# areanddee/Sharding-the-Sphere-Fall-2025-JAX-DevLab-Examples

Measured on AMD Instinct MI355X. Metric: cell-updates/sec (whole node) at C96, higher is better.
Workload: dtype fp64; 1 GPU; global_batch=1, seq_len=55296, parallelism=spatial tiles: 24 tiles over 1 GPU(s), auto partition, N=96, tiles_per_edge=2, integrator=ssprk3, backend=hip, comm=none, steps_per_launch=6, fused_block=16, graph_replayed_steps=0, direct_launch_steps=1662, kernel_launches=277, eager_steps=0

## Files before the change

### sharding-the-sphere-fall-2025-jax-devlab-examples_amd/ops/csrc/fused_step.hip

```cpp
#include "stage_common.h"

#include <type_traits>


#ifndef STSP_FPROBE_ALLEDGE
#define STSP_FPROBE_ALLEDGE 0
#endif
#ifndef STSP_XG_FENCE
#define STSP_XG_FENCE 0
#endif
#ifndef STSP_FUSED_TAGH
#define STSP_FUSED_TAGH 1
#endif
#ifndef STSP_FUSED_TAIL_OWN
#define STSP_FUSED_TAIL_OWN 1
#endif
#ifndef STSP_FUSED_POLL2
#define STSP_FUSED_POLL2 1
#endif
#ifndef STSP_FUSED_RF_MINB
#define STSP_FUSED_RF_MINB 12
#endif

namespace {
// ... 10 lines not shown
  static constexpr int WW = GB + GMAX;
  static constexpr int L1 = R - 2 * (NS - 1);
  static constexpr int H1 = B + 4 * (NS - 1);
  static constexpr int NFX = H1 * (H1 + 1);
  static constexpr int NFL = 2 * NFX;
  static constexpr int NU = H1 * H1;
  static constexpr int NT = NU <= 768 ? 768 : 1024;
  static_assert(NU <= NT && W * W <= 2 * NT, "owner threads for every updated cell");
  static constexpr int NTAIL = W * W > NT ? W * W - NT : 0;
  static constexpr int NTO = STSP_FUSED_TAIL_OWN ? B * B : NT - NU;
  static constexpr int TPT = NTAIL ? (NTAIL + NTO - 1) / NTO : 1;
  static_assert(GMAX <= NT, "one fix-up thread per ghost entry");
  static_assert(2 * (B + 4 * (NS - 2)) * (B + 4 * (NS - 2) + 1) <= 32 * 64 && 2 * H1 * (H1 + 1) <= 32 * 64 + 64 * 64,
                "face passes per stage fit the 32-entry pass table");
  static constexpr int CMAX = 32;
};

__device__ __forceinline__ int fregion(int X, int Y, int N) {
  const bool inx = (unsigned)X < (unsigned)N, iny = (unsigned)Y < (unsigned)N;
  if (inx) return iny ? 0 : (Y < 0 ? 3 : 4);
  return iny ? (X < 0 ? 1 : 2) : -1;
}

__host__ __device__ __forceinline__ constexpr void annulus(int t, int lo, int L, int w, int& u, int& v) {
  if (t < w * L) {
    u = lo + t % L; v = lo + t / L;
    return;
  }
  t -= w * L;
  if (t < w * L) {
// ... 88 lines not shown
  unsigned mdiv_n;
  T a0[4], a1[4], a2[4];
  T dt, g, omega2;
  int ring, K;
  const unsigned long long* recv;
  T* const* peer_ring;
  const int* xpush;
  int* epoch;
  int* err;
  long long timeout_ticks;
  unsigned long long* stamps;
  int nsteps;
  const int* prod;
  int PM;
  const unsigned* sched;
  const T* nrmf;
  unsigned long long* hx;
  const signed char* pidx;
};

__device__ __forceinline__ void fused_fail(int* err, unsigned code, int bid, int xe, int what, int seen) {
  if (atomicCAS((unsigned*)err, 0u, code) == 0u) {
    __hip_atomic_store(err + 1, bid, __ATOMIC_RELAXED, __HIP_MEMORY_SCOPE_AGENT);
    __hip_atomic_store(err + 2, xe, __ATOMIC_RELAXED, __HIP_MEMORY_SCOPE_AGENT);
    __hip_atomic_store(err + 3, what, __ATOMIC_RELAXED, __HIP_MEMORY_SCOPE_AGENT);
    __hip_atomic_store(err + 4, seen, __ATOMIC_RELAXED, __HIP_MEMORY_SCOPE_AGENT);
  }
}

template <class C, int SCOPE, bool FENCE = false, class Fail>
// ... 82 lines not shown

template <typename T>
__device__ __forceinline__ T pair_swap(T v) {
  if constexpr (sizeof(T) == 8) {
    int2 p = __builtin_bit_cast(int2, v);
    p.x = __builtin_amdgcn_update_dpp(0, p.x, 0xB1, 0xF, 0xF, false);
    p.y = __builtin_amdgcn_update_dpp(0, p.y, 0xB1, 0xF, 0xF, false);
    return __builtin_bit_cast(T, p);
  } else {
    return __builtin_bit_cast(T, __builtin_amdgcn_update_dpp(0, __builtin_bit_cast(int, v), 0xB1, 0xF, 0xF, false));
  }
}

__device__ __forceinline__ int sel5(int r, int v0, int v1, int v2, int v3, int v4) {
  return r == 0 ? v0 : r == 1 ? v1 : r == 2 ? v2 : r == 3 ? v3 : v4;
}

__device__ __forceinline__ int ncode(unsigned long long c, int side) {
  return (int)(short)(unsigned short)(c >> (16 * side));
}

template <typename T, int LIM, int NS, int B, bool XG, bool MULTI>
__global__ __launch_bounds__((FD<NS, B>::NT)) void fused_step_kernel(FArgs<T> a) {
  using D = FD<NS, B>;
  constexpr int W = D::W, WS = D::WS, WW = D::WW, GB = D::GB, R = D::R, L1 = D::L1, H1 = D::H1;
  constexpr int NFX = D::NFX, NFL = D::NFL, NT = D::NT;
  static_assert(window_covered_once<NS, B>(), "owner and tail cells cover the window exactly once");
  constexpr bool RING_FIRST = B >= STSP_FUSED_RF_MINB;
  constexpr bool PFN = sizeof(T) == 4 || B <= 16;
  constexpr int NRG = PFN ? 1 : 5;
  constexpr int NN = 2 * NRG * 3 * (W + 1);
  __shared__ T s_w[5 * WW];
  __shared__ T s_fl[4][NFL];
  __shared__ T s_len[NFL];
  __shared__ T s_nrm[2][NRG][3][W + 1];
  __shared__ T s_nrmf[PFN ? 3 * NFL : 1];
  constexpr int CS = W + 1;
  __shared__ unsigned long long s_code[W * CS];
  __shared__ short s_gs[D::GMAX][2];
  __shared__ T s_gt[D::GMAX];
  __shared__ int s_ct[D::CMAX][CT_INTS];
  __shared__ T s_cg[D::CMAX][CG_VALS];
  constexpr int NX2 = NS > 1 ? (B + 4 * (NS - 2)) * (B + 4 * (NS - 2)) : 1;
  __shared__ T s_x[4][NX2];
  __shared__ int s_gdone;

  const int tid = threadIdx.x;
  const int bid = xcd_remap(blockIdx.x, a.nblocks);
  const int N = a.N;
  const int* og = a.org + bid * 4;
  const int X0 = og[0], Y0 = og[1], tile = og[2], ow = og[3];
  const int xo = ow & 0xFFF, yo = (ow >> 12) & 0xFFF, flags = (ow >> 24) & 0x1F;
  const bool edge = (flags & 0x1E) != 0;
  const int ngw = edge ? (a.G + 63) >> 6 : 0;
  int gbase = 0;
  int gtarget = 0;
  if (tid == 0) s_gdone = 0;
  const T* wf = &s_w[0];
  FSTAMP(0);
  FSTAMP_RT(14);
// ... 41 lines not shown
      gs1 = a.gtab[((long)bid * a.G + tid) * 2 + 1];
      gtv = a.gw[(long)bid * a.G + tid];
    }
    ncor = a.ccnt[bid];
    gbase = 64 * (ncor > 0 ? 1 : 0);
    if (tid < ncor) {
      const int* ct = a.ctab + ((long)bid * a.C + tid) * CT_INTS;
      const T* cg = a.cgf + ((long)bid * a.C + tid) * CG_VALS;
#pragma unroll
      for (int k = 0; k < CT_INTS; ++k) ctv[k] = ct[k];
#pragma unroll
      for (int k = 0; k < CG_VALS; ++k) cgv[k] = cg[k];
    }
  }
  const int wv = __builtin_amdgcn_readfirstlane(tid >> 6);
  unsigned pmask[3], nmask[3];
#pragma unroll
  for (int s = 0; s < 3; ++s) {
    pmask[s] = __builtin_amdgcn_readfirstlane(a.sched[((long)bid * 3 + s) * 17 + wv]);
    nmask[s] = __builtin_amdgcn_readfirstlane(a.sched[((long)bid * 3 + s) * 17 + 16]);
  }
  constexpr int LPT = (NFL + NT - 1) / NT;
  T lnv[LPT];
  if (flags == 1) {
#pragma unroll
    for (int k = 0; k < LPT; ++k) {
      const int j = tid + k * NT;
      const bool yf = j >= NFX;
      const int jj = yf ? j - NFX : j;
      const int r = yf ? jj / H1 : jj / (H1 + 1), c = yf ? jj - r * H1 : jj - r * (H1 + 1);
      const int li = yf ? (X0 + L1 + c) * (N + 1) + Y0 + L1 + r : (Y0 + L1 + r) * (N + 1) + X0 + L1 + c;
      lnv[k] = j < NFL ? a.lxt[li] : T(0);
    }
  } else {
#pragma unroll
// ... 138 lines not shown
      to_global((int)(a.frames >> (9 * ((unsigned)ow >> 29))) & 511, ax ? T(0) : rn, ax ? rn : T(0), -nrv * rn,
                m0, m1, m2);
      s_nrm[ax][0][0][k] = m0; s_nrm[ax][0][1][k] = m1; s_nrm[ax][0][2][k] = m2;
    } else {
      (&s_nrm[0][0][0][0])[tid] = nrv;
    }
  }
  if (!PFN && NN > NT && flags != 1 && tid + NT < NN) (&s_nrm[0][0][0][0])[tid + NT] = nrv2;
  if (PFN && flags != 1) {
#pragma unroll
    for (int k = 0; k < NPF; ++k) {
      const int j = tid + k * NT;
      if (j < 3 * NFL) s_nrmf[j] = nfv[k];
    }
  }
  if (edge) {
    if (owner) s_code[v * CS + u] = cdv;
    if (tid < a.G) { s_gs[tid][0] = (short)gs0; s_gs[tid][1] = (short)gs1; s_gt[tid] = gtv; }
    if (tid < ncor) {
#pragma unroll
      for (int k = 0; k < CT_INTS; ++k) s_ct[tid][k] = ctv[k];
#pragma unroll
      for (int k = 0; k < CG_VALS; ++k) s_cg[tid][k] = cgv[k];
    }
  }
  auto put_at = [&](int wi, const T (&q)[4]) {
    const T inv = q[0] != T(0) ? trcp(q[0]) : T(0);
    T* p = &s_w[0] + wi;
    p[0] = q[0];
    p[WW] = q[1] * inv;
// ... 72 lines not shown
      wl[f] = cl[f] + half_slope<LIM>(cl[f] - am, ap - cl[f]);
      wr[f] = cr[f] - half_slope<LIM>(cr[f] - bm, bp - cr[f]);
    }
    T m0, m1, m2;
    if constexpr (MODE != 0 && PFN) {
      m0 = s_nrmf[fslot]; m1 = s_nrmf[NFL + fslot]; m2 = s_nrmf[2 * NFL + fslot];
    } else {
      const T* m = &s_nrm[ax ? 1 : 0][ra][0][k];
      m0 = m[0]; m1 = m[W + 1]; m2 = m[2 * (W + 1)];
    }
    T fl[4];
    swe_flux<T>(wl, wr, cl, cr, m0, m1, m2, s_len[fslot], a.g, fl);
#pragma unroll
    for (int f = 0; f < 4; ++f) s_fl[f][fslot] = fl[f];
  };
  constexpr int NIL = B - 3, NI = 2 * NIL * B;
  constexpr int OL0 = R + 2 - L1, OL1 = (W - L1) - (R + B - 1) + 1;
  constexpr int NR1 = H1, NOR = H1 - B;
  constexpr int NOA = (OL0 + OL1) * NR1, NOX = NOA + NIL * NOR;
  static_assert(NOX + NIL * B == H1 * (H1 + 1), "inner + outer = the stage-1 face set");
  auto inner_face = [&](int t) {
    const bool ax = t >= NIL * B;
    const int t2 = ax ? t - NIL * B : t;
    const int k = R + 2 + t2 / B, p = R + t2 % B;
    if (PFN && edge) {
      if (ax) face(true, p, k, k, std::integral_constant<int, 1>{});
      else face(false, k, p, k, std::integral_constant<int, 1>{});
    } else {
      if (ax) face(true, p, k, k, std::integral_constant<int, 0>{});
      else face(false, k, p, k, std::integral_constant<int, 0>{});
// ... 16 lines not shown
      for (int f = 0; f < 4; ++f) s_x[f][tid] = Q[f];
    }
    if (owner) put(Q);
  };

  for (int it = 0; it < nsteps; ++it) {
  FSTAMP(13);
  const bool wait = MULTI && it > 0;
  if (wait) {
    if (tid < B * B) enter_cell();
  } else {
    enter_cell();
  }
  __syncthreads();
  if (wait && !tagh && !pcell && tid < 64) {
    const int p = tid < a.PM ? a.prod[(long)bid * a.PM + tid] : -1;
    const int pa = p >= 0 ? p : bid;
    bool ok = false;
    xg_spin(a.err, a.timeout_ticks, [&] {
      const int e = __hip_atomic_load(a.epoch + pa, __ATOMIC_RELAXED, __HIP_MEMORY_SCOPE_AGENT);
      ok = p < 0 || e >= xe;
      return __builtin_amdgcn_ballot_w64(!ok) == 0;
    }, [&] {
      if (!ok) fused_fail(a.err, 2u, bid, xe, p, __hip_atomic_load(a.epoch + p, __ATOMIC_RELAXED,
                                                                    __HIP_MEMORY_SCOPE_AGENT));
    });
  } else {
    const bool w0 = wait && !tagh && !pcell;
    const bool rf = RING_FIRST && wait && tagh;
    const int t0 = w0 ? tid - 64 : (rf ? (tid < B * B ? B * B - 1 - tid : NI) : tid);
    const int dt_ = w0 ? NT - 64 : (rf ? B * B : NT);
// ... 1 lines not shown
  }
  FSTAMP(1);
  if (!(wait && (tagh || pcell))) __syncthreads();
  if (wait) {
    T tq[TPT][4];
    if (tagh) {
      tail_load_tagged(xe, tq);
      if (tid >= B * B) {
        if (src >= 0) load_tagged(src, Q, xe);
        else load_state_of(src, Q, nullptr, xe);
        enter_cell();
      }
    } else {
      if (pcell) {
        auto poll_prod = [&](int cu, int cv) {
          const int k = a.pidx[(long)bid * W * W + cv * W + cu];
          if (k < 0) return;
          const int p = a.prod[(long)bid * a.PM + k];
          int e = 0;
          xg_spin(a.err, a.timeout_ticks, [&] {
            e = __hip_atomic_load(a.epoch + p, __ATOMIC_RELAXED, __HIP_MEMORY_SCOPE_AGENT);
            return e >= xe;
          }, [&] { fused_fail(a.err, 2u, bid, xe, p, e); });
        };
        if (tid >= B * B && owner) poll_prod(u, v);
#pragma unroll
        for (int k = 0; k < TPT; ++k)
          if (tl_wi[k] >= 0) poll_prod(tl_wi[k] % WS, tl_wi[k] / WS);
      }
      tail_load(buf[it & 1], xe, tq);
      if (tid >= B * B) {
// ... 21 lines not shown
          const T x0 = wf[f * WW + i0], x1 = wf[f * WW + i1];
          s_w[f * WW + GB + ge] = x0 + t * (x1 - x0);
        }
      }
      if (ge >= 0 && ge < ngw * 64 && (tid & 63) == 0) {
        asm volatile("s_waitcnt lgkmcnt(0)" ::: "memory");
        __hip_atomic_fetch_add(&s_gdone, 1, __ATOMIC_RELEASE, __HIP_MEMORY_SCOPE_WORKGROUP);
      }
      gtarget += ngw;
    }
    const int nax = s == 0 ? NOX : nx;
    const int ntask = 2 * nax;
    unsigned m = pmask[s];
    for (int first = (ncor && wv == 0) ? 1 : 0; first || m;) {
      int task;
      bool nearp = false;
      if (first) {
        task = (tid & 63) - 64;
        first = 0;
      } else {
        const int pp = __builtin_ctz(m);
        task = pp * 64 + (tid & 63);
        nearp = (nmask[s] >> pp) & 1u;
        m &= m - 1u;
      }
      if (task >= ntask) continue;
      if (task >= 0) {
        const int tf = task;
        const bool ax = tf >= nax;
        const int t2 = ax ? tf - nax : tf;
        int fu, fv, k, p;
        if (s == 0) {
          outer_face(t2, k, p);
        } else {
          const int c = t2 / nr, r = t2 - c * nr;
          k = lo + c; p = lo + r;
        }
        if (!ax) { fv = p; fu = k; }
        else { fu = p; fv = k; }
        if (edge || STSP_FPROBE_ALLEDGE) {
          if (PFN && !nearp) face(ax, fu, fv, k, std::integral_constant<int, 1>{});
          else face(ax, fu, fv, k, std::integral_constant<int, 2>{});
// ... 95 lines not shown
      for (int f = 0; f < 4; ++f) {
        T* p = o32(Out, so + f * S);
        if constexpr (sizeof(T) == 8)
          __hip_atomic_store((gu64*)p, __builtin_bit_cast(unsigned long long, Q[f]), __ATOMIC_RELAXED,
                             __HIP_MEMORY_SCOPE_AGENT);
        else
          __hip_atomic_store((gu32*)p, __builtin_bit_cast(unsigned, Q[f]), __ATOMIC_RELAXED,
                             __HIP_MEMORY_SCOPE_AGENT);
      }
    } else {
#pragma unroll
      for (int f = 0; f < 4; ++f) *o32(Out, so + f * S) = Q[f];
    }
    if (last) {
      const int n = a.n, mg = a.mg;
      const int x = xo + u - R, y = yo + v - R;
      const int* pm = a.push + (long)tile * 4 * mg * n;
      int pt[4] = {-1, -1, -1, -1};
      if (x < mg) pt[0] = pm[(0 * mg + x) * n + y];
      if (x >= n - mg) pt[1] = pm[(1 * mg + (n - 1 - x)) * n + y];
      if (y < mg) pt[2] = pm[(2 * mg + y) * n + x];
      if (y >= n - mg) pt[3] = pm[(3 * mg + (n - 1 - y)) * n + x];
      if (a.cpush && (x < mg || x >= n - mg) && (y < mg || y >= n - mg)) {
        const int qx = x < mg ? 0 : 1, qy = y < mg ? 0 : 1;
        const int c = a.cpush[((tile * 4 + (qx | (qy << 1))) * mg + (qy ? n - 1 - y : y)) * mg + (qx ? n - 1 - x : x)];
        if (c != -1) pt[qx ^ 1] = c;
      }
#pragma unroll
      for (int k = 0; k < 4; ++k) {
        if (pt[k] >= 0) {
#pragma unroll
// ... 53 lines not shown
    a.a0[k] = (T)d->a0[k]; a.a1[k] = (T)d->a1[k]; a.a2[k] = (T)d->a2[k];
  }
  a.dt = (T)d->dt; a.g = (T)d->g; a.omega2 = (T)d->omega2;
  a.ring = d->ring; a.K = d->K; a.recv = (const unsigned long long*)d->recv; a.peer_ring = (T* const*)d->peer_ring;
  a.xpush = d->xpush; a.epoch = d->epoch; a.err = d->err; a.timeout_ticks = d->timeout_ticks;
  a.stamps = d->stamps;
  for (int k = 0; k < 6; ++k) a.links[k] = d->links[k];
  a.local_src = d->local_src;
  a.nsteps = d->nsteps < 1 ? 1 : d->nsteps;
  a.prod = d->prod;
  a.PM = d->PM;
  a.sched = (const unsigned*)d->sched;
  a.nrmf = (const T*)d->nrmf;
  a.hx = (unsigned long long*)d->hx;
  a.pidx = d->pidx;
  if (!a.sched || !a.nrmf) return -4;
  if (a.nsteps > 1 && (!a.prod || a.PM <= 0 || a.PM > 64 || !d->epoch || !d->err)) return -7;
  a.mdiv_n = magic_div((unsigned)d->n, (unsigned long long)d->N + 1);
  if (d->xg && (!d->recv || !d->peer_ring || !d->xpush || !d->epoch || !d->err || d->ring <= 0 ||
                d->K <= 0))
    return -6;
  const dim3 grid(d->nblocks), block(D::NT);
  if (d->limiter < 0 || d->limiter > 3) return -4;
  if (a.nsteps > 1) {
    static int cdev[2][4] = {{-1, -1, -1, -1}, {-1, -1, -1, -1}}, ccap[2][4] = {};
    int dev = 0;
    if (hipGetDevice(&dev) != hipSuccess) return -8;
    const int xi = d->xg ? 1 : 0, li = d->limiter;
    if (cdev[xi][li] != dev) {
      int cus = 0, per = 0;
      if (hipDeviceGetAttribute(&cus, hipDeviceAttributeMultiprocessorCount, dev) != hipSuccess) return -8;
// ... 76 lines not shown
extern "C" int stsp_fused_prime_launch(int dtype, const void* q, int S, const int* src, const int* code, int nent,
                                       void* const* peer_ring, int ring, int epoch, hipStream_t stream) {
  if (nent <= 0) return 0;
  const dim3 grid((nent + 255) / 256), block(256);
  if (dtype == 1)
    hipLaunchKernelGGL(fused_prime_kernel<double>, grid, block, 0, stream, (const double*)q, S, src, code, nent,
                       (double* const*)peer_ring, ring, epoch);
  else if (dtype == 0)
    hipLaunchKernelGGL(fused_prime_kernel<float>, grid, block, 0, stream, (const float*)q, S, src, code, nent,
                       (float* const*)peer_ring, ring, epoch);
  else
    return -4;
  return (int)hipGetLastError();
}

extern "C" int stsp_fused_tagh(void) { return STSP_FUSED_TAGH; }

extern "C" int stsp_fused_limits(int* gmax, int* cmax) {
  *gmax = FD<3, 16>::GMAX;
  *cmax = FD<3, 16>::CMAX;
  return 0;
}
```

### sharding-the-sphere-fall-2025-jax-devlab-examples_amd/ops/csrc/stsp_kernels.h

```cpp
#pragma once
#include <hip/hip_runtime.h>
#include <stdint.h>

extern "C" {

typedef struct StageDesc {
  const void* X;
  const void* Q;
  const void* acc_in;
  void* out;
  void* acc_out;
  const void* recv;
  const int* gmap;
  const int* push;
  const int* blocks;
  const void* invA;
  const void* ex;
  const void* ey;
  const void* mx;
  const void* my;
  const void* cgeo;
  int ntile, n, S, mg, pw;
  int nblocks;
  int limiter;
// ... 73 lines not shown
  int K;
  int* epoch;
  int* err;
  long long timeout_ticks;
  unsigned long long* stamps;
  int local_src;
  int links[6];
  int nsteps;
  const int* prod;
  int PM;
  const int* cpush;
  const unsigned* sched;
  const void* nrmf;
  void* hx;
  const signed char* pidx;
} FusedDesc;
int stsp_fused_launch(int dtype, const FusedDesc* d, hipStream_t stream);
int stsp_fused_limits(int* gmax, int* cmax);
int stsp_fused_tagh(void);
int stsp_fused_record_words(int dtype);
int stsp_fused_prime_launch(int dtype, const void* q, int S, const int* src, const int* code, int nent,
                            void* const* peer_ring, int ring, int epoch, hipStream_t stream);
typedef struct DerivedDesc {
  const void* Q;
  const void* recv;
  const int* gmap;
  const int* cgmap;
  const int* pedge;
  const int* pe_base;
  const void* pe_t;
  const void* cdx;
  const void* cdy;
  const void* mx;
  const void* my;
// ... 180 lines not shown
```

### sharding-the-sphere-fall-2025-jax-devlab-examples_amd/ops/fused.py

```python
from __future__ import annotations

import hashlib
import os
from dataclasses import dataclass
from typing import Dict, List, Optional, Tuple

import numpy as np
import torch

from ..models.base import panel_edge_tables
from ..parallel.layout import TileLayout, ghost_xy
from ..parallel.topology import neighbor_cells


def native_stream(device) -> int:
    from .native import current_stream_handle
    return current_stream_handle(device)

REG_P, REG_W, REG_E, REG_S, REG_N = 0, 1, 2, 3, 4
NREG = 5
SIDE_VEC = ((-1, 0), (1, 0), (0, -1), (0, 1))
NG_PLR = 2


# ... 735 lines not shown


def stage_face_counts(B: int, ns: int = 3) -> List[int]:
    h1 = B + 4 * (ns - 1)
    nil = B - 3
    out = [2 * (h1 * (h1 + 1) - nil * B)]
    for s in range(1, ns):
        nr = B + 4 * (ns - 1 - s)
        out.append(2 * nr * (nr + 1))
    return out


PASS_SLOTS = 32


def pass_schedule(B: int, ncorner: np.ndarray, edge: np.ndarray, G: int, ns: int = 3,
                  weights: Optional[str] = None) -> np.ndarray:
    import os
    weights = weights or os.environ.get("STSP_FUSED_SCHED", "5:1")
    nt = fused_threads(B, ns)
    nw = nt // 64
    counts = stage_face_counts(B, ns)
    nb = len(ncorner)
    out = np.zeros((nb, ns, PASS_SLOTS), dtype=np.uint8)
    ngw = -(-G // 64) if G > 0 else 0
    cache = {}
    for b in range(nb):
        cw = 1 if ncorner[b] > 0 else 0
        gw = ngw if edge[b] else 0
        key = (cw, gw)
        if key not in cache:
            tab = np.zeros((ns, PASS_SLOTS), dtype=np.uint8)
            for s, nt_s in enumerate(counts):
                npass = -(-nt_s // 64)
                assert npass <= PASS_SLOTS
                if weights == "legacy":
                    first = nw - cw
                    for p in range(npass):
                        tab[s, p] = p + cw if p < first else cw + gw + (p - first) % (nw - cw - gw)
                    continue
                wc, wg = (int(x) for x in weights.split(":"))
                wl = [0] * nw
                if cw:
                    wl[0] += wc
                for w in range(cw, cw + gw):
                    wl[w] += wg
                for p in range(npass):
                    gl = [sum(wl[w] for w in range(g, nw, 4)) for g in range(4)]
                    g = min(range(4), key=lambda g_: (gl[g_], g_))
                    w = min(range(g, nw, 4), key=lambda w_: (wl[w_], w_))
                    tab[s, p] = w
                    wl[w] += 4
            cache[key] = tab
        out[b] = cache[key]
    return out


def pass_masks(B: int, sched: np.ndarray, ns: int = 3, near: Optional[np.ndarray] = None) -> np.ndarray:
    counts = stage_face_counts(B, ns)
    nb = sched.shape[0]
    m = np.zeros((nb, ns, 17), dtype=np.uint32)
    for s_, cnt in enumerate(counts):
        for p in range(-(-cnt // 64)):
            w = sched[:, s_, p].astype(np.int64)
            m[np.arange(nb), s_, w] |= np.uint32(1 << p)
    if near is not None:
        m[:, :, 16] = near
# ... 70 lines not shown
    fu = L1 + c
    fv = L1 + r
    k = np.where(yf, fv, fu)
    lu = fu - np.where(yf, 0, 1)
    lv = fv - np.where(yf, 1, 0)
    ax = yf.astype(np.int64)
    out = np.zeros((P.nb, 3, nfl))
    for b in range(P.nb):
        if flags[b] == 1:
            continue
        X0, Y0 = int(P.org[b, 0]), int(P.org[b, 1])
        ra = region(X0 + lu, Y0 + lv, P.N)
        ra = np.where(ra < 0, 0, ra)
        out[b] = P.nrm[b, ax, ra, k, :].T
    return out


def fused_supported(engine, B: Optional[int] = None) -> Optional[str]:
    e = engine
    return fused_supported_config(e.physics, e.integ.name, e.layout, B)


def fused_supported_config(physics, integrator: str, layout: TileLayout, B: Optional[int] = None) -> Optional[str]:
    from ..models.swe import ShallowWater
    if not isinstance(physics, ShallowWater):
        return "fused step: shallow water only"
    if getattr(physics, "kernel_id", None) == 4:
        return "fused step: no layers"
    if physics.F != 4:
        return "fused step: no tracers"
# ... 114 lines not shown
        if self.handoff == "tag" and not int(self.lib.stsp_fused_tagh()):
            if os.environ.get("STSP_FUSED_HANDOFF") == "tag":
                raise RuntimeError("STSP_FUSED_HANDOFF=tag needs a library built with STSP_FUSED_TAGH=1")
            self.handoff = "epoch"
        if self.handoff == "tag":
            words = 5 if e.dtype == torch.float64 else 4
            self.tens["hx"] = torch.zeros(2 * words * e.plan.S, dtype=torch.int64, device=dev)
        self.tens["err"] = torch.zeros(8, dtype=torch.int32, device=dev)
        prod = producer_table(P)
        self.tens["prod"] = torch.as_tensor(prod, dtype=torch.int32, device=dev).contiguous()
        self.poll = poll_mode() if (X is None and self.handoff == "epoch" and read_relation_symmetric(P)) \
            else "block"
        if self.poll == "cell":
            self.tens["pidx"] = torch.as_tensor(cell_producer_index(P, prod), device=dev).contiguous()
        edge_b = np.array([any(int(x) > 0 for x in np.unique(P.reg[b])) for b in range(nb)])
        sched = pass_schedule(B, np.asarray(P.ccnt), edge_b, G)
        assert int(sched.max()) < fused_threads(B) // 64
        flg = (org[:, 3].view(np.uint32) >> 24) & 0x1F
        near = near_pass_masks(B, P.org, flg.astype(np.int64), e.layout.N)
        self.tens["sched"] = torch.as_tensor(pass_masks(B, sched, near=near).view(np.int32), device=dev).contiguous()
        self.tens["nrmf"] = t(face_normals(P, flg.astype(np.int64)))
        self.timeout_ticks = int(timeout_s * 1e8)
        if X is not None:
            self._setup_exchange(X, timeout_s)
        self.descs = [self._desc(0, 1), self._desc(1, 0)]
        self._multi = {}
        self._multi_ptrs = {}
        if X is not None:
            self.prime()

    def _setup_exchange(self, X, timeout_s: float) -> None:
        from .xgmi import IpcRing, _declare, refuse_if_forced
        refuse_if_forced()
        e = self.e
        L = _declare(self.lib)
# ... 39 lines not shown
        d.dt = e.dt
        d.g = float(e.physics.g)
        d.omega2 = 2.0 * float(e.physics.omega)
        d.local_src = 1 if (self.world == 1 and not e.layout.loopback
                            and list(e.plan.tiles) == list(range(e.layout.num_tiles))) else 0
        for f in range(6):
            d.links[f] = face_links(f)
        d.epoch = p(tn["epoch"])
        d.err = p(tn["err"])
        d.timeout_ticks = self.timeout_ticks
        d.nsteps = nsteps
        d.prod = p(tn["prod"])
        d.PM = int(tn["prod"].shape[1])
        d.sched = p(tn["sched"])
        d.nrmf = p(tn["nrmf"])
        d.hx = p(tn["hx"]) if self.handoff == "tag" else 0
        d.pidx = p(tn["pidx"]) if self.poll == "cell" else 0
        if self.mem is not None:
            d.xg = 1
            d.ring = self.ring
            d.recv = self.mem.base
            d.peer_ring = p(tn["peer_ring"])
            d.xpush = p(tn["xpush"])
            d.K = self.K
        return d

    def multi_desc(self, nsteps: int):
        if nsteps < 2 or nsteps % 2:
            raise ValueError("a multi-step launch runs an even number of steps")
        d = self._multi.get(nsteps)
# ... 318 lines not shown
```

### sharding-the-sphere-fall-2025-jax-devlab-examples_amd/ops/native.py

```python
from __future__ import annotations

import ctypes
import os
import threading

import torch

from . import build as _build

_LIB = None
_LOCK = threading.Lock()


class StageDesc(ctypes.Structure):
    _fields_ = [
        ("X", ctypes.c_void_p), ("Q", ctypes.c_void_p), ("acc_in", ctypes.c_void_p),
        ("out", ctypes.c_void_p), ("acc_out", ctypes.c_void_p), ("recv", ctypes.c_void_p),
        ("gmap", ctypes.c_void_p), ("push", ctypes.c_void_p), ("blocks", ctypes.c_void_p),
        ("invA", ctypes.c_void_p), ("ex", ctypes.c_void_p), ("ey", ctypes.c_void_p),
        ("mx", ctypes.c_void_p), ("my", ctypes.c_void_p), ("cgeo", ctypes.c_void_p),
        ("ntile", ctypes.c_int), ("n", ctypes.c_int), ("S", ctypes.c_int), ("mg", ctypes.c_int), ("pw", ctypes.c_int),
        ("nblocks", ctypes.c_int), ("limiter", ctypes.c_int), ("remote", ctypes.c_int),
        ("a0", ctypes.c_double), ("a1", ctypes.c_double), ("a2", ctypes.c_double),
        ("c0", ctypes.c_double), ("c1", ctypes.c_double), ("c2", ctypes.c_double), ("dt", ctypes.c_double),
# ... 18 lines not shown
        ("code", ctypes.c_void_p),
        ("gtab", ctypes.c_void_p), ("gw", ctypes.c_void_p), ("ctab", ctypes.c_void_p), ("cgf", ctypes.c_void_p),
        ("ccnt", ctypes.c_void_p), ("push", ctypes.c_void_p),
        ("G", ctypes.c_int), ("C", ctypes.c_int),
        ("nblocks", ctypes.c_int), ("n", ctypes.c_int), ("N", ctypes.c_int), ("S", ctypes.c_int),
        ("mg", ctypes.c_int), ("pw", ctypes.c_int), ("B", ctypes.c_int), ("ns", ctypes.c_int),
        ("limiter", ctypes.c_int),
        ("a0", ctypes.c_double * 4), ("a1", ctypes.c_double * 4), ("a2", ctypes.c_double * 4),
        ("dt", ctypes.c_double), ("g", ctypes.c_double), ("omega2", ctypes.c_double),
        ("xg", ctypes.c_int), ("ring", ctypes.c_int), ("recv", ctypes.c_void_p), ("peer_ring", ctypes.c_void_p),
        ("xpush", ctypes.c_void_p), ("K", ctypes.c_int), ("epoch", ctypes.c_void_p), ("err", ctypes.c_void_p),
        ("timeout_ticks", ctypes.c_longlong), ("stamps", ctypes.c_void_p),
        ("local_src", ctypes.c_int), ("links", ctypes.c_int * 6),
        ("nsteps", ctypes.c_int), ("prod", ctypes.c_void_p), ("PM", ctypes.c_int),
        ("cpush", ctypes.c_void_p), ("sched", ctypes.c_void_p), ("nrmf", ctypes.c_void_p),
        ("hx", ctypes.c_void_p), ("pidx", ctypes.c_void_p),
    ]


class March3Desc(ctypes.Structure):
    _fields_ = [
        ("q1", ctypes.c_void_p), ("q2", ctypes.c_void_p),
        ("b0", ctypes.c_double * 3), ("b1", ctypes.c_double * 3), ("b2", ctypes.c_double * 3),
        ("D", ctypes.c_int),
    ]


class DerivedDesc(ctypes.Structure):
    _fields_ = [
        ("Q", ctypes.c_void_p), ("recv", ctypes.c_void_p), ("gmap", ctypes.c_void_p), ("cgmap", ctypes.c_void_p),
        ("pedge", ctypes.c_void_p), ("pe_base", ctypes.c_void_p), ("pe_t", ctypes.c_void_p),
# ... 85 lines not shown
            except Exception:
                if not os.path.exists(path):
                    raise
        L = ctypes.CDLL(path, mode=ctypes.RTLD_GLOBAL)
        vp, ci, cl = ctypes.c_void_p, ctypes.c_int, ctypes.c_long
        L.stsp_pack_launch.argtypes = [ci, vp, ci, ci, vp, ci, vp, vp]
        L.stsp_pack_launch.restype = ci
        L.stsp_copy_index_launch.argtypes = [ci, vp, vp, vp, vp, ci, ci, cl, cl, vp]
        L.stsp_copy_index_launch.restype = ci
        L.stsp_dpp_probe.argtypes = [vp, vp, vp, vp]
        L.stsp_dpp_probe.restype = ci
        L.stsp_fused_limits.argtypes = [ctypes.POINTER(ci), ctypes.POINTER(ci)]
        L.stsp_fused_limits.restype = ci
        L.stsp_fused_tagh.argtypes = []
        L.stsp_fused_tagh.restype = ci
        L.stsp_fused_record_words.argtypes = [ci]
        L.stsp_fused_record_words.restype = ci
        L.stsp_fused_prime_launch.argtypes = [ci, vp, ci, vp, vp, ci, vp, ci, ci, vp]
        L.stsp_fused_prime_launch.restype = ci
        for launch, argtypes, cls, (query, args) in DESCRIPTORS:
            fn, size = getattr(L, launch), getattr(L, query)
            fn.argtypes, fn.restype = argtypes, ci
            size.argtypes, size.restype = [ci] * len(args), ci
            if size(*args) != ctypes.sizeof(cls):
                raise RuntimeError(f"{cls.__name__}: ctypes mirror is {ctypes.sizeof(cls)} bytes, "
                                   f"the library's {size(*args)} (stale libstsp.so?)")
        L.stsp_stage_batch_launch.argtypes = [ci, ci, ci, ci, _P(StageDesc), ci, ctypes.c_longlong, vp]
        L.stsp_stage_batch_launch.restype = ci
        _declare_runtime(L)
        _declare_tt(L)
# ... 145 lines not shown
```

Before: 4.889 billion cell-updates/s.

## Drive face passes from a per-class task table with lane-shared slopes

Replaces the arithmetic task-to-face mapping in the fused step with a host-built per-block-class face table in shared memory. Interior faces are grouped into contiguous runs along each line, so adjacent lanes compute one limited half-slope each and pass it to the neighbour with a DPP row shift, instead of every face recomputing both slopes. Passes are load-balanced across waves with per-pass weights. The cost is extra LDS for the table, a table load per block, idle and slope-only slots at run boundaries, and added host scheduling complexity.

```diff
diff --git a/sharding-the-sphere-fall-2025-jax-devlab-examples_amd/ops/csrc/fused_step.hip b/sharding-the-sphere-fall-2025-jax-devlab-examples_amd/ops/csrc/fused_step.hip
--- a/sharding-the-sphere-fall-2025-jax-devlab-examples_amd/ops/csrc/fused_step.hip
+++ b/sharding-the-sphere-fall-2025-jax-devlab-examples_amd/ops/csrc/fused_step.hip
@@ -48,6 +48,11 @@
   static_assert(2 * (B + 4 * (NS - 2)) * (B + 4 * (NS - 2) + 1) <= 32 * 64 && 2 * H1 * (H1 + 1) <= 32 * 64 + 64 * 64,
                 "face passes per stage fit the 32-entry pass table");
   static constexpr int CMAX = 32;
+  static constexpr int cdiv64(int x) { return (x + 63) / 64; }
+  static constexpr int TCAP = cdiv64(2 * (H1 * (H1 + 1) - (B - 3) * B)) + 2 +
+                              (NS > 1 ? cdiv64(2 * (B + 4 * (NS - 2)) * (B + 4 * (NS - 2) + 1)) + 2 : 0) +
+                              (NS > 2 ? cdiv64(2 * (B + 4 * (NS - 3)) * (B + 4 * (NS - 3) + 1)) + 2 : 0);
+  static_assert(NS <= 3, "TCAP sums three stages");
 };
 
 __device__ __forceinline__ int fregion(int X, int Y, int N) {
@@ -166,6 +171,7 @@
   const int* prod;
   int PM;
   const unsigned* sched;
+  const unsigned short* ftab;
   const T* nrmf;
   unsigned long long* hx;
   const signed char* pidx;
@@ -278,6 +284,19 @@
 
 __device__ __forceinline__ int sel5(int r, int v0, int v1, int v2, int v3, int v4) {
   return r == 0 ? v0 : r == 1 ? v1 : r == 2 ? v2 : r == 3 ? v3 : v4;
+}
+
+template <typename T>
+__device__ __forceinline__ T next_lane(T v) {
+  if constexpr (sizeof(T) == 8) {
+    int2 p = __builtin_bit_cast(int2, v);
+    p.x = __builtin_amdgcn_update_dpp(p.x, p.x, 0x130, 0xF, 0xF, false);
+    p.y = __builtin_amdgcn_update_dpp(p.y, p.y, 0x130, 0xF, 0xF, false);
+    return __builtin_bit_cast(T, p);
+  } else {
+    const int x = __builtin_bit_cast(int, v);
+    return __builtin_bit_cast(T, __builtin_amdgcn_update_dpp(x, x, 0x130, 0xF, 0xF, false));
+  }
 }
 
 __device__ __forceinline__ int ncode(unsigned long long c, int side) {
@@ -308,6 +327,8 @@
   constexpr int NX2 = NS > 1 ? (B + 4 * (NS - 2)) * (B + 4 * (NS - 2)) : 1;
   __shared__ T s_x[4][NX2];
   __shared__ int s_gdone;
+  constexpr int NTB = PFN ? 64 * D::TCAP : 2;
+  __shared__ unsigned short s_tab[NTB];
 
   const int tid = threadIdx.x;
   const int bid = xcd_remap(blockIdx.x, a.nblocks);
@@ -379,11 +400,15 @@
     }
   }
   const int wv = __builtin_amdgcn_readfirstlane(tid >> 6);
-  unsigned pmask[3], nmask[3];
+  unsigned pmask[3], nmask[3], smask[3];
+  int tb[3];
 #pragma unroll
   for (int s = 0; s < 3; ++s) {
-    pmask[s] = __builtin_amdgcn_readfirstlane(a.sched[((long)bid * 3 + s) * 17 + wv]);
-    nmask[s] = __builtin_amdgcn_readfirstlane(a.sched[((long)bid * 3 + s) * 17 + 16]);
+    const unsigned* sw = a.sched + ((long)bid * 3 + s) * 20;
+    pmask[s] = __builtin_amdgcn_readfirstlane(sw[wv]);
+    nmask[s] = __builtin_amdgcn_readfirstlane(sw[16]);
+    smask[s] = PFN ? __builtin_amdgcn_readfirstlane(sw[17]) : 0u;
+    tb[s] = PFN ? __builtin_amdgcn_readfirstlane(sw[18]) : 0;
   }
   constexpr int LPT = (NFL + NT - 1) / NT;
   T lnv[LPT];
@@ -552,6 +577,10 @@
       if (j < 3 * NFL) s_nrmf[j] = nfv[k];
     }
   }
+  if constexpr (PFN) {
+    const unsigned* tp = (const unsigned*)a.ftab + (long)a.sched[(long)bid * 3 * 20 + 19] * (NTB / 2);
+    for (int j = tid; j < NTB / 2; j += NT) ((unsigned*)s_tab)[j] = tp[j];
+  }
   if (edge) {
     if (owner) s_code[v * CS + u] = cdv;
     if (tid < a.G) { s_gs[tid][0] = (short)gs0; s_gs[tid][1] = (short)gs1; s_gt[tid] = gtv; }
@@ -654,6 +683,41 @@
 #pragma unroll
     for (int f = 0; f < 4; ++f) s_fl[f][fslot] = fl[f];
   };
+  auto face_shared = [&](bool ax, int fu, int fv, int k, bool flux, auto mode_c) {
+    constexpr int MODE = decltype(mode_c)::value;
+    const int st = ax ? WS : 1;
+    int fslot = ax ? NFX + (k - L1) * H1 + (fu - L1) : (fv - L1) * (H1 + 1) + (k - L1);
+    fslot = flux ? fslot : 0;
+    const int ib = fv * WS + fu, ia = ib - st, iam = ia - st;
+    T cl[5], cr[5], hsa[4], hsb[4];
+#pragma unroll
+    for (int f = 0; f < 5; ++f) { cl[f] = wf[f * WW + ia]; cr[f] = wf[f * WW + ib]; }
+#pragma unroll
+    for (int f = 0; f < 4; ++f) {
+      const T am = wf[f * WW + iam];
+      hsa[f] = half_slope<LIM>(cl[f] - am, cr[f] - cl[f]);
+    }
+#pragma unroll
+    for (int f = 0; f < 4; ++f) hsb[f] = next_lane(hsa[f]);
+    if (!flux) return;
+    T wl[4], wr[4];
+#pragma unroll
+    for (int f = 0; f < 4; ++f) {
+      wl[f] = cl[f] + hsa[f];
+      wr[f] = cr[f] - hsb[f];
+    }
+    T m0, m1, m2;
+    if constexpr (MODE != 0) {
+      m0 = s_nrmf[fslot]; m1 = s_nrmf[NFL + fslot]; m2 = s_nrmf[2 * NFL + fslot];
+    } else {
+      const T* m = &s_nrm[ax ? 1 : 0][0][0][k];
+      m0 = m[0]; m1 = m[W + 1]; m2 = m[2 * (W + 1)];
+    }
+    T fl[4];
+    swe_flux<T>(wl, wr, cl, cr, m0, m1, m2, s_len[fslot], a.g, fl);
+#pragma unroll
+    for (int f = 0; f < 4; ++f) s_fl[f][fslot] = fl[f];
+  };
   constexpr int NIL = B - 3, NI = 2 * NIL * B;
   constexpr int OL0 = R + 2 - L1, OL1 = (W - L1) - (R + B - 1) + 1;
   constexpr int NR1 = H1, NOR = H1 - B;
@@ -700,7 +764,9 @@
   }
   __syncthreads();
   if (wait && !tagh && !pcell && tid < 64) {
-    const int p = tid < a.PM ? a.prod[(long)bid * a.PM + tid] : -1;
+    int pt = tid;
+    asm volatile("" : "+v"(pt));
+    const int p = tid < a.PM ? a.prod[(long)bid * a.PM + pt] : -1;
     const int pa = p >= 0 ? p : bid;
     bool ok = false;
     xg_spin(a.err, a.timeout_ticks, [&] {
@@ -732,7 +798,9 @@
     } else {
       if (pcell) {
         auto poll_prod = [&](int cu, int cv) {
-          const int k = a.pidx[(long)bid * W * W + cv * W + cu];
+          int ci = cv * W + cu;
+          asm volatile("" : "+v"(ci));
+          const int k = a.pidx[(long)bid * W * W + ci];
           if (k < 0) return;
           const int p = a.prod[(long)bid * a.PM + k];
           int e = 0;
@@ -784,7 +852,7 @@
     unsigned m = pmask[s];
     for (int first = (ncor && wv == 0) ? 1 : 0; first || m;) {
       int task;
-      bool nearp = false;
+      bool nearp = false, sharep = false;
       if (first) {
         task = (tid & 63) - 64;
         first = 0;
@@ -792,10 +860,27 @@
         const int pp = __builtin_ctz(m);
         task = pp * 64 + (tid & 63);
         nearp = (nmask[s] >> pp) & 1u;
+        sharep = (smask[s] >> pp) & 1u;
         m &= m - 1u;
       }
-      if (task >= ntask) continue;
-      if (task >= 0) {
+      if (!PFN && task >= ntask) continue;
+      if (PFN && task >= 0) {
+        const unsigned e = s_tab[tb[s] * 64 + task];
+        const int fu = e & 31, fv = (e >> 5) & 31, kind = (e >> 11) & 3;
+        const bool ax = (e >> 10) & 1;
+        const int k = ax ? fv : fu;
+        if (sharep) {
+          if (edge || STSP_FPROBE_ALLEDGE) face_shared(ax, fu, fv, k, kind == 1, std::integral_constant<int, 1>{});
+          else face_shared(ax, fu, fv, k, kind == 1, std::integral_constant<int, 0>{});
+        } else if (kind == 2) {
+          if (edge || STSP_FPROBE_ALLEDGE) {
+            if (!nearp) face(ax, fu, fv, k, std::integral_constant<int, 1>{});
+            else face(ax, fu, fv, k, std::integral_constant<int, 2>{});
+          } else {
+            face(ax, fu, fv, k, std::integral_constant<int, 0>{});
+          }
+        }
+      } else if (task >= 0) {
         const int tf = task;
         const bool ax = tf >= nax;
         const int t2 = ax ? tf - nax : tf;
@@ -921,7 +1006,8 @@
     }
     if (last) {
       const int n = a.n, mg = a.mg;
-      const int x = xo + u - R, y = yo + v - R;
+      int x = xo + u - R, y = yo + v - R;
+      asm volatile("" : "+v"(x), "+v"(y));
       const int* pm = a.push + (long)tile * 4 * mg * n;
       int pt[4] = {-1, -1, -1, -1};
       if (x < mg) pt[0] = pm[(0 * mg + x) * n + y];
@@ -1005,7 +1091,8 @@
   a.nrmf = (const T*)d->nrmf;
   a.hx = (unsigned long long*)d->hx;
   a.pidx = d->pidx;
-  if (!a.sched || !a.nrmf) return -4;
+  a.ftab = (const unsigned short*)d->ftab;
+  if (!a.sched || !a.nrmf || !a.ftab) return -4;
   if (a.nsteps > 1 && (!a.prod || a.PM <= 0 || a.PM > 64 || !d->epoch || !d->err)) return -7;
   a.mdiv_n = magic_div((unsigned)d->n, (unsigned long long)d->N + 1);
   if (d->xg && (!d->recv || !d->peer_ring || !d->xpush || !d->epoch || !d->err || d->ring <= 0 ||
@@ -1112,6 +1199,18 @@
   return (int)hipGetLastError();
 }
 
+extern "C" int stsp_fused_table_passes(int B) {
+  switch (B) {
+    case 6: return FD<3, 6>::TCAP;
+    case 8: return FD<3, 8>::TCAP;
+    case 12: return FD<3, 12>::TCAP;
+    case 16: return FD<3, 16>::TCAP;
+    case 18: return FD<3, 18>::TCAP;
+    case 20: return FD<3, 20>::TCAP;
+    default: return 0;
+  }
+}
+
 extern "C" int stsp_fused_tagh(void) { return STSP_FUSED_TAGH; }
 
 extern "C" int stsp_fused_limits(int* gmax, int* cmax) {
diff --git a/sharding-the-sphere-fall-2025-jax-devlab-examples_amd/ops/csrc/stsp_kernels.h b/sharding-the-sphere-fall-2025-jax-devlab-examples_amd/ops/csrc/stsp_kernels.h
--- a/sharding-the-sphere-fall-2025-jax-devlab-examples_amd/ops/csrc/stsp_kernels.h
+++ b/sharding-the-sphere-fall-2025-jax-devlab-examples_amd/ops/csrc/stsp_kernels.h
@@ -111,10 +111,12 @@
   const void* nrmf;
   void* hx;
   const signed char* pidx;
+  const unsigned short* ftab;
 } FusedDesc;
 int stsp_fused_launch(int dtype, const FusedDesc* d, hipStream_t stream);
 int stsp_fused_limits(int* gmax, int* cmax);
 int stsp_fused_tagh(void);
+int stsp_fused_table_passes(int B);
 int stsp_fused_record_words(int dtype);
 int stsp_fused_prime_launch(int dtype, const void* q, int S, const int* src, const int* code, int nent,
                             void* const* peer_ring, int ring, int epoch, hipStream_t stream);
diff --git a/sharding-the-sphere-fall-2025-jax-devlab-examples_amd/ops/fused.py b/sharding-the-sphere-fall-2025-jax-devlab-examples_amd/ops/fused.py
--- a/sharding-the-sphere-fall-2025-jax-devlab-examples_amd/ops/fused.py
+++ b/sharding-the-sphere-fall-2025-jax-devlab-examples_amd/ops/fused.py
@@ -773,6 +773,31 @@
 PASS_SLOTS = 32
 
 
+def _balance_passes(npasses: List[int], nw: int, cw: int, gw: int, weights: str,
+                    loads: Optional[List[List[int]]] = None) -> np.ndarray:
+    tab = np.zeros((len(npasses), PASS_SLOTS), dtype=np.uint8)
+    for s, npass in enumerate(npasses):
+        assert npass <= PASS_SLOTS
+        if weights == "legacy":
+            first = nw - cw
+            for p in range(npass):
+                tab[s, p] = p + cw if p < first else cw + gw + (p - first) % (nw - cw - gw)
+            continue
+        wc, wg = (int(x) for x in weights.split(":")[:2])
+        wl = [0] * nw
+        if cw:
+            wl[0] += wc
+        for w in range(cw, cw + gw):
+            wl[w] += wg
+        for p in range(npass):
+            gl = [sum(wl[w] for w in range(g, nw, 4)) for g in range(4)]
+            g = min(range(4), key=lambda g_: (gl[g_], g_))
+            w = min(range(g, nw, 4), key=lambda w_: (wl[w_], w_))
+            tab[s, p] = w
+            wl[w] += loads[s][p] if loads is not None else 4
+    return tab
+
+
 def pass_schedule(B: int, ncorner: np.ndarray, edge: np.ndarray, G: int, ns: int = 3,
                   weights: Optional[str] = None) -> np.ndarray:
     import os
@@ -789,27 +814,7 @@
         gw = ngw if edge[b] else 0
         key = (cw, gw)
         if key not in cache:
-            tab = np.zeros((ns, PASS_SLOTS), dtype=np.uint8)
-            for s, nt_s in enumerate(counts):
-                npass = -(-nt_s // 64)
-                assert npass <= PASS_SLOTS
-                if weights == "legacy":
-                    first = nw - cw
-                    for p in range(npass):
-                        tab[s, p] = p + cw if p < first else cw + gw + (p - first) % (nw - cw - gw)
-                    continue
-                wc, wg = (int(x) for x in weights.split(":"))
-                wl = [0] * nw
-                if cw:
-                    wl[0] += wc
-                for w in range(cw, cw + gw):
-                    wl[w] += wg
-                for p in range(npass):
-                    gl = [sum(wl[w] for w in range(g, nw, 4)) for g in range(4)]
-                    g = min(range(4), key=lambda g_: (gl[g_], g_))
-                    w = min(range(g, nw, 4), key=lambda w_: (wl[w_], w_))
-                    tab[s, p] = w
-                    wl[w] += 4
+            tab = _balance_passes([-(-c // 64) for c in counts], nw, cw, gw, weights)
             cache[key] = tab
         out[b] = cache[key]
     return out
@@ -910,6 +915,159 @@
         ra = np.where(ra < 0, 0, ra)
         out[b] = P.nrm[b, ax, ra, k, :].T
     return out
+
+
+FT_IDLE, FT_SHARED, FT_FULL, FT_SLOPE = 0, 1, 2, 3
+FT_MIN_RUN = 3
+SHARE_LOADS = (3, 6)
+SCHED_WORDS = 20
+
+
+def ft_pack(ax, fu, fv, kind):
+    return (np.asarray(fu) | (np.asarray(fv) << 5) | (np.asarray(ax) << 10) | (np.asarray(kind) << 11)).astype(np.uint16)
+
+
+def ft_unpack(e):
+    e = np.asarray(e).astype(np.int64)
+    fu, fv, ax, kind = e & 31, (e >> 5) & 31, (e >> 10) & 1, (e >> 11) & 3
+    return ax, np.where(ax == 1, fv, fu), np.where(ax == 1, fu, fv), kind
+
+
+def share_enabled() -> bool:
+    return os.environ.get("STSP_FUSED_SHARE", "1") != "0"
+
+
+def fused_pfn(B: int, fp32: bool) -> bool:
+    return fp32 or B <= 16
+
+
+def block_class(flags: int) -> Tuple[int, int]:
+    return (int(flags) >> 1) & 3, (int(flags) >> 3) & 3
+
+
+def class_edge_lines(B: int, cls: Tuple[int, int], ns: int = 3) -> Tuple[List[int], List[int]]:
+    R = 2 * ns
+    return tuple([R + B * j for j in range(2) if c >> j & 1] for c in cls)
+
+
+def table_pass_cap(B: int, ns: int = 3) -> int:
+    return sum(-(-c // 64) + 2 for c in stage_face_counts(B, ns))
+
+
+def _pack_runs(runs: List[Tuple[int, int, List[int]]]) -> List[Tuple[int, int, int, int]]:
+    slots: List[Tuple[int, int, int, int]] = []
+    idle = (0, 0, 0, FT_IDLE)
+    for ax, p, ks in runs:
+        ks = list(ks)
+        while ks:
+            rem = 64 - len(slots) % 64
+            if len(ks) + 1 <= rem:
+                take = len(ks)
+            else:
+                take = min(rem - 1, len(ks) - FT_MIN_RUN)
+                if take < FT_MIN_RUN:
+                    slots += [idle] * rem
+                    continue
+            slots += [(ax, k, p, FT_SHARED) for k in ks[:take]]
+            slots.append((ax, ks[take - 1] + 1, p, FT_SLOPE))
+            ks = ks[take:]
+    slots += [idle] * (-len(slots) % 64)
+    return slots
+
+
+def face_table(B: int, cls: Tuple[int, int], ns: int = 3, share: Optional[bool] = None):
+    share = share_enabled() if share is None else share
+    d = FusedDims.make(B, ns)
+    lines = class_edge_lines(B, cls, ns)
+    out = []
+    for ax, k, p in stage_face_coords(B, ns):
+        near = np.zeros(len(k), bool)
+        for a_ in range(2):
+            for e in lines[a_]:
+                near |= (ax == a_) & (np.abs(k - e) <= 1)
+        if not share:
+            full = list(range(len(k)))
+            slots = []
+        else:
+            rows: Dict[Tuple[int, int], List[int]] = {}
+            for t in np.flatnonzero(~near):
+                rows.setdefault((int(ax[t]), int(p[t])), []).append(int(k[t]))
+            runs, short = [], set()
+            for (a_, p_), ks in sorted(rows.items()):
+                ks.sort()
+                cut = [0] + [i for i in range(1, len(ks)) if ks[i] != ks[i - 1] + 1] + [len(ks)]
+                for i0, i1 in zip(cut[:-1], cut[1:]):
+                    if i1 - i0 >= FT_MIN_RUN:
+                        runs.append((a_, p_, ks[i0:i1]))
+                    else:
+                        short.update((a_, k_, p_) for k_ in ks[i0:i1])
+            slots = _pack_runs(runs)
+            idx = np.arange(len(k))
+            full = list(idx[near]) + [t for t in idx[~near] if (int(ax[t]), int(k[t]), int(p[t])) in short]
+        fslots = [(int(ax[t]), int(k[t]), int(p[t]), FT_FULL) for t in full]
+        fslots += [(0, 0, 0, FT_IDLE)] * (-len(fslots) % 64)
+        nfull = len(fslots) // 64
+        slots = fslots + slots
+        sa, sk, sp, kind = (np.array(x, np.int64) for x in zip(*slots))
+        idle = kind == FT_IDLE
+        sk[idle], sp[idle] = d.L1 + 1, d.L1
+        ent = ft_pack(sa, np.where(sa == 1, sp, sk), np.where(sa == 1, sk, sp), kind)
+        npass = len(slots) // 64
+        assert npass <= PASS_SLOTS
+        nearset = set(zip(ax[near].tolist(), k[near].tolist(), p[near].tolist()))
+        nm = 0
+        for q in range(nfull):
+            if any(s_[3] == FT_FULL and s_[:3] in nearset for s_ in slots[64 * q:64 * q + 64]):
+                nm |= 1 << q
+        out.append((ent, nm, ((1 << npass) - 1) & ~((1 << nfull) - 1)))
+    return out
+
+
+def pass_loads(tabs, weights: str) -> List[List[int]]:
+    f = weights.split(":")
+    wsh, wnear = (int(f[2]), int(f[3])) if len(f) >= 4 else SHARE_LOADS
+    return [[wnear if (nm >> q) & 1 else wsh if (sm >> q) & 1 else 4 for q in range(len(ent) // 64)]
+            for ent, nm, sm in tabs]
+
+
+def face_tables(B: int, flags: np.ndarray, ncorner: np.ndarray, edge: np.ndarray, G: int, ns: int = 3,
+                share: Optional[bool] = None, weights: Optional[str] = None):
+    weights = weights or os.environ.get("STSP_FUSED_SCHED", "5:1")
+    nw = fused_threads(B, ns) // 64
+    cap = table_pass_cap(B, ns)
+    ngw = -(-G // 64) if G > 0 else 0
+    nb = len(flags)
+    classes = sorted(set(block_class(f) for f in flags))
+    ftab = np.zeros((len(classes), 64 * cap), dtype=np.uint16)
+    per_class = {}
+    for ci, cls in enumerate(classes):
+        tabs = face_table(B, cls, ns, share)
+        off = 0
+        offs = []
+        for ent, _, _ in tabs:
+            offs.append(off)
+            ftab[ci, 64 * off:64 * off + len(ent)] = ent
+            off += len(ent) // 64
+        if off > cap:
+            raise RuntimeError(f"fused step: {off} face passes of block class {cls} exceed the kernel's table ({cap})")
+        per_class[cls] = (ci, tabs, offs)
+    sched = np.zeros((nb, ns, SCHED_WORDS), dtype=np.uint32)
+    cache = {}
+    for b in range(nb):
+        cls = block_class(flags[b])
+        key = (cls, 1 if ncorner[b] > 0 else 0, ngw if edge[b] else 0)
+        if key not in cache:
+            ci, tabs, offs = per_class[cls]
+            wave = _balance_passes([len(t[0]) // 64 for t in tabs], nw, key[1], key[2], weights,
+                                   pass_loads(tabs, weights) if weights != "legacy" else None)
+            m = np.zeros((ns, SCHED_WORDS), dtype=np.uint32)
+            for s_, (ent, nm, sm) in enumerate(tabs):
+                for q in range(len(ent) // 64):
+                    m[s_, wave[s_, q]] |= np.uint32(1 << q)
+                m[s_, 16], m[s_, 17], m[s_, 18], m[s_, 19] = nm, sm, offs[s_], ci
+            cache[key] = m
+        sched[b] = cache[key]
+    return ftab, sched, classes
 
 
 def fused_supported(engine, B: Optional[int] = None) -> Optional[str]:
@@ -1054,11 +1212,27 @@
         if self.poll == "cell":
             self.tens["pidx"] = torch.as_tensor(cell_producer_index(P, prod), device=dev).contiguous()
         edge_b = np.array([any(int(x) > 0 for x in np.unique(P.reg[b])) for b in range(nb)])
-        sched = pass_schedule(B, np.asarray(P.ccnt), edge_b, G)
-        assert int(sched.max()) < fused_threads(B) // 64
         flg = (org[:, 3].view(np.uint32) >> 24) & 0x1F
-        near = near_pass_masks(B, P.org, flg.astype(np.int64), e.layout.N)
-        self.tens["sched"] = torch.as_tensor(pass_masks(B, sched, near=near).view(np.int32), device=dev).contiguous()
+        self.pfn = fused_pfn(B, e.dtype == torch.float32)
+        if self.pfn:
+            R_ = d.R
+            for b in range(nb):
+                X0, Y0 = int(P.org[b, 0]), int(P.org[b, 1])
+                kx = [k for f_, k in ((2, -X0), (4, e.layout.N - X0)) if flg[b] & f_]
+                ky = [k for f_, k in ((8, -Y0), (16, e.layout.N - Y0)) if flg[b] & f_]
+                assert (kx, ky) == tuple(class_edge_lines(B, block_class(flg[b]))), (b, kx, ky, R_)
+            ftab, sched20, self.classes = face_tables(B, flg.astype(np.int64), np.asarray(P.ccnt), edge_b, G)
+            assert ftab.shape[1] == 64 * int(self.lib.stsp_fused_table_passes(B))
+        else:
+            sched = pass_schedule(B, np.asarray(P.ccnt), edge_b, G)
+            assert int(sched.max()) < fused_threads(B) // 64
+            near = near_pass_masks(B, P.org, flg.astype(np.int64), e.layout.N)
+            sched20 = np.zeros((nb, 3, SCHED_WORDS), dtype=np.uint32)
+            sched20[:, :, :17] = pass_masks(B, sched, near=near)
+            ftab = np.zeros((1, 64), dtype=np.uint16)
+        assert int(np.log2(np.maximum(sched20[:, :, :16].max(), 1))) < PASS_SLOTS
+        self.tens["sched"] = torch.as_tensor(sched20.view(np.int32), device=dev).contiguous()
+        self.tens["ftab"] = torch.as_tensor(ftab.view(np.int16), device=dev).contiguous()
         self.tens["nrmf"] = t(face_normals(P, flg.astype(np.int64)))
         self.timeout_ticks = int(timeout_s * 1e8)
         if X is not None:
@@ -1128,6 +1302,7 @@
         d.PM = int(tn["prod"].shape[1])
         d.sched = p(tn["sched"])
         d.nrmf = p(tn["nrmf"])
+        d.ftab = p(tn["ftab"])
         d.hx = p(tn["hx"]) if self.handoff == "tag" else 0
         d.pidx = p(tn["pidx"]) if self.poll == "cell" else 0
         if self.mem is not None:
diff --git a/sharding-the-sphere-fall-2025-jax-devlab-examples_amd/ops/native.py b/sharding-the-sphere-fall-2025-jax-devlab-examples_amd/ops/native.py
--- a/sharding-the-sphere-fall-2025-jax-devlab-examples_amd/ops/native.py
+++ b/sharding-the-sphere-fall-2025-jax-devlab-examples_amd/ops/native.py
@@ -56,7 +56,7 @@
         ("local_src", ctypes.c_int), ("links", ctypes.c_int * 6),
         ("nsteps", ctypes.c_int), ("prod", ctypes.c_void_p), ("PM", ctypes.c_int),
         ("cpush", ctypes.c_void_p), ("sched", ctypes.c_void_p), ("nrmf", ctypes.c_void_p),
-        ("hx", ctypes.c_void_p), ("pidx", ctypes.c_void_p),
+        ("hx", ctypes.c_void_p), ("pidx", ctypes.c_void_p), ("ftab", ctypes.c_void_p),
     ]
 
 
@@ -172,6 +172,8 @@
         L.stsp_fused_limits.restype = ci
         L.stsp_fused_tagh.argtypes = []
         L.stsp_fused_tagh.restype = ci
+        L.stsp_fused_table_passes.argtypes = [ci]
+        L.stsp_fused_table_passes.restype = ci
         L.stsp_fused_record_words.argtypes = [ci]
         L.stsp_fused_record_words.restype = ci
         L.stsp_fused_prime_launch.argtypes = [ci, vp, ci, vp, vp, ci, vp, ci, ci, vp]
```

Measured after the change: 5.119 billion cell-updates/s, median of 6. 1.05x the previous value.
